# MariMamgo/CNN-with-PDE

Hardware: AMD Instinct MI355X
Metric: PDE-layer fwd+bwd Msamples/s (higher is better)
Workload: dtype f32; 1 GPU; cifar10.EnhancedDiffusionLayer(size=32, channels=64, num_steps=10) fwd+bwd, 30 implicit sweeps, batch 512/GPU, channel mixing disabled (BASELINE configs[1], SURVEY §8d cfg2 primary); global_batch=512, parallelism=dp1, grad_allreduce_bytes=0, rccl_world_size=1

## Files before the change

### cnn-with-pde_amd/_lib.py

```python
import ctypes as C
import os

HERE = os.path.dirname(os.path.abspath(__file__))
LIB_PATH = os.environ.get("PDECNN_LIB") or os.path.join(HERE, "lib", "libpdecnn_hip.so")

PDE_MAX_SWEEPS = 96
PDE_MAX_N = 32
PDE_MAX_N_GENERIC = 128
PDE_IO_F32, PDE_IO_BF16, PDE_IO_F64, PDE_IO_F16 = 0, 1, 2, 3
PDE_AXIS_X, PDE_AXIS_Y = 0, 1
PDE_MIX_PATH_SCALAR, PDE_MIX_PATH_MFMA_F32, PDE_MIX_PATH_MFMA_16, PDE_MIX_PATH_SPLIT3, PDE_MIX_PATH_FUSED = 0, 1, 2, 3, 4
PDE_RH_PATH_STRIP32, PDE_RH_PATH_STRIP16, PDE_RH_PATH_ROW_BLOCKS = 0, 1, 2
PDE_RH_DK_SPLIT3, PDE_RH_DK_MFMA_F32 = 0, 1
PDE_JACOBI_MAX_HW = 1024
PDE_JACOBI_TILED_K = 10

ERRORS = {
    -1: "PDE_E_BADARG (null pointer, bad dimension or enum)",
    -2: "PDE_E_UNSUPPORTED_N (line length — either side of a rectangle — outside [2, 128], or a per-step / one-launch "
        "entry point at a line length without fused kernels: those exist for multiples of 4 in [8, 32])",
    -3: "PDE_E_TOO_MANY_SWEEPS",
    -4: "PDE_E_LAUNCH (HIP launch failed)",
    -5: "PDE_E_WORKSPACE (workspace too small or misaligned)",
}


class PdeSweep(C.Structure):
    _fields_ = [("axis", C.c_int32), ("delta", C.c_float), ("h2", C.c_float), ("t", C.c_float)]


class PdeAdiDesc(C.Structure):
    _fields_ = [("B", C.c_int32), ("C", C.c_int32), ("N", C.c_int32), ("io_dtype", C.c_int32),
                ("num_sweeps", C.c_int32), ("smooth3", C.c_int32), ("has_clamp_max", C.c_int32),
                ("clamp_max", C.c_float), ("eps", C.c_float), ("sweep", PdeSweep * PDE_MAX_SWEEPS)]


class PdeSweepF64(C.Structure):
    _fields_ = [("axis", C.c_int32), ("pad", C.c_int32), ("delta", C.c_double), ("h2", C.c_double), ("t", C.c_double)]


class PdeAdiDescF64(C.Structure):
    _fields_ = [("B", C.c_int32), ("C", C.c_int32), ("N", C.c_int32), ("io_dtype", C.c_int32),
                ("num_sweeps", C.c_int32), ("smooth3", C.c_int32), ("has_clamp_max", C.c_int32), ("pad", C.c_int32),
                ("clamp_max", C.c_double), ("eps", C.c_double), ("sweep", PdeSweepF64 * PDE_MAX_SWEEPS)]


class PdeAdiRectDesc(C.Structure):
    _fields_ = [("B", C.c_int32), ("C", C.c_int32), ("H", C.c_int32), ("W", C.c_int32), ("io_dtype", C.c_int32),
                ("num_sweeps", C.c_int32), ("smooth3", C.c_int32), ("has_clamp_max", C.c_int32),
                ("clamp_max", C.c_float), ("eps", C.c_float), ("sweep", PdeSweep * PDE_MAX_SWEEPS)]


class PdeAdiRectDescF64(C.Structure):
    _fields_ = [("B", C.c_int32), ("C", C.c_int32), ("H", C.c_int32), ("W", C.c_int32), ("io_dtype", C.c_int32),
                ("num_sweeps", C.c_int32), ("smooth3", C.c_int32), ("has_clamp_max", C.c_int32),
                ("clamp_max", C.c_double), ("eps", C.c_double), ("sweep", PdeSweepF64 * PDE_MAX_SWEEPS)]


class PdeSmallLayer(C.Structure):
    _fields_ = [("desc", C.POINTER(PdeAdiDesc)), ("sweeps_per_step", C.c_int32), ("mode", C.c_int32),
                ("M", C.c_void_p), ("skip_weight", C.c_void_p),
                ("alpha_base", C.c_void_p), ("beta_base", C.c_void_p), ("alpha_slope", C.c_void_p), ("beta_slope", C.c_void_p),
                ("weight", C.c_float), ("weight_ptr", C.c_void_p), ("states", C.c_void_p), ("plane_sums", C.c_void_p),
                ("steps_workspace", C.c_void_p), ("steps_workspace_bytes", C.c_size_t),
                ("kappa_max", C.c_void_p), ("kappa_max_host", C.c_void_p),
                ("gys", C.c_void_p), ("g_plane_sums", C.c_void_p), ("ckpt_mask", C.POINTER(C.c_uint64)),
                ("g_alpha_base", C.c_void_p), ("g_beta_base", C.c_void_p), ("g_alpha_slope", C.c_void_p),
                ("g_beta_slope", C.c_void_p), ("gM", C.c_void_p), ("g_skip_weight", C.c_void_p), ("g_weight", C.c_void_p),
                ("workspace", C.c_void_p), ("workspace_bytes", C.c_size_t)]


class PdeError(RuntimeError):
    pass


_vp, _fp, _sz, _i32, _f32, _f64 = C.c_void_p, C.c_void_p, C.c_size_t, C.c_int32, C.c_float, C.c_double
_D = C.POINTER(PdeAdiDesc)
_D64 = C.POINTER(PdeAdiDescF64)
_DR = C.POINTER(PdeAdiRectDesc)
_DR64 = C.POINTER(PdeAdiRectDescF64)

SIGNATURES = {
    "pde_adi_line_length_path": (C.c_int, [_i32]),
    "pde_adi_forward_kernel": (C.c_int, [C.POINTER(PdeAdiDesc)]),
    "pde_adi_backward_kernel": (C.c_int, [C.POINTER(PdeAdiDesc), _i32]),
    "pde_adi_forward_workspace_bytes": (_sz, [_D]),
    "pde_adi_backward_workspace_bytes": (_sz, [_D, _i32]),
    "pde_adi_forward": (C.c_int, [_D, _vp, _vp, _fp, _fp, _fp, _fp, _fp, _fp, _vp, _vp, _sz, _vp]),
    "pde_adi_backward": (C.c_int, [_D, _vp, _vp, _vp, C.POINTER(C.c_uint64), _vp, _fp, _fp, _fp, _fp,
                                   _fp, _fp, _fp, _fp, _vp, _vp, _sz, _vp]),
    "pde_adi_forward_states": (C.c_int, [_D, _vp, _vp, _vp, C.POINTER(C.c_uint64), _fp, _fp, _fp, _fp, _fp, _fp, _vp, _vp,
                                         _sz, _vp]),
    "pde_adi_backward_states": (C.c_int, [_D, _vp, _vp, C.POINTER(C.c_uint64), _vp, _vp, C.POINTER(C.c_uint64), _vp,
                                          _fp, _fp, _fp, _fp, _fp, _fp, _fp, _fp, _vp, _vp, _sz, _vp]),
    "pde_adi_kappa_max": (C.c_int, [_D, _fp, _fp, _fp, _fp, _fp, _vp]),
    "pde_adi_steps_workspace_bytes": (_sz, [_D, _i32]),
    "pde_adi_factor_steps": (C.c_int, [_D, _i32, _fp, _fp, _fp, _fp, _fp, _vp, _sz, _vp]),
    "pde_adi_forward_step": (C.c_int, [_D, _i32, _i32, _vp, _vp, _vp, _vp]),
    "pde_adi_backward_step_workspace_bytes": (_sz, [_D, _i32, _i32]),
    "pde_adi_backward_step": (C.c_int, [_D, _i32, _i32, _vp, _vp, _vp, C.POINTER(C.c_uint64), _vp, _vp, _vp, _sz,
                                        _i32, _vp]),
    "pde_adi_param_grads": (C.c_int, [_D, _i32, _fp, _fp, _fp, _fp, _fp, _fp, _fp, _fp, _vp, _vp, _vp]),
    "pde_adi_mixed_forward": (C.c_int, [_D, _i32, _i32, _vp, _vp, _vp, _fp, _fp, _fp, _fp, _fp, _fp, _fp, _vp, _vp, _sz, _vp]),
    "pde_adi_mixed_backward_workspace_bytes": (_sz, [_D, _i32, _i32]),
    "pde_adi_mixed_backward": (C.c_int, [_D, _i32, _i32, _vp, _vp, _vp, _vp, _fp, C.POINTER(C.c_uint64), _vp, _fp, _fp, _fp, _fp,
                                         _fp, _fp, _fp, _fp, _fp, _vp, _vp, _sz, _vp]),
    "pde_adi_small_supported": (C.c_int, [_D, _i32]),
    "pde_adi_mixed_one_launch": (C.c_int, [_D, _i32]),
    "pde_adi_small_forward": (C.c_int, [_D, _i32, _i32, _vp, _vp, _vp, _fp, _fp, _fp, _fp, _fp, _fp, _fp, _fp, _vp, _vp, _sz,
                                        _vp]),
    "pde_adi_small_backward_workspace_bytes": (_sz, [_D, _i32, _i32]),
    "pde_adi_small_backward": (C.c_int, [_D, _i32, _i32, _vp, _vp, _vp, _fp, _fp, C.POINTER(C.c_uint64), _vp,
                                         _fp, _fp, _fp, _fp, _fp, _fp, _fp, _fp, _fp, _fp, _vp, _vp, _sz, _vp]),
    "pde_adi_small_forward_states": (C.c_int, [_D, _i32, _i32, _vp, _vp, _vp, _vp, C.POINTER(C.c_uint64), _fp, _fp, _fp, _fp,
                                               _fp, _fp, _fp, _vp, _vp, _sz, _vp]),
    "pde_adi_small_backward_states": (C.c_int, [_D, _i32, _i32, _vp, _vp, C.POINTER(C.c_uint64), _vp, _vp, _fp,
                                                C.POINTER(C.c_uint64), _vp, _fp, _fp, _fp, _fp, _fp, _fp, _fp, _fp, _fp,
                                                _vp, _vp, _sz, _vp]),
    "pde_adi_multi_forward": (C.c_int, [_i32, C.POINTER(PdeSmallLayer), _vp, _vp, _vp, _vp]),
    "pde_adi_multi_backward": (C.c_int, [_i32, C.POINTER(PdeSmallLayer), _vp, _vp, _vp, _vp]),
    "pde_gate_combine_forward": (C.c_int, [_i32, _i32, _i32, _i32, _i32, C.POINTER(C.c_void_p), C.POINTER(C.c_void_p), _fp,
                                           _vp, _vp]),
    "pde_gate_combine_backward": (C.c_int, [_i32, _i32, _i32, _i32, _i32, _vp, C.POINTER(C.c_void_p), C.POINTER(C.c_void_p),
                                            _fp, C.POINTER(C.c_void_p), C.POINTER(C.c_void_p), _vp]),
    "pde_bn_pool_workspace_bytes": (_sz, [_i32, _i32]),
    "pde_bn_pool_forward": (C.c_int, [_i32, _i32, _i32, _fp, _fp, _fp, _f32, _i32, _f32, _fp, _fp, _fp, _fp, _fp, _vp, _vp, _sz,
                                      _vp]),
    "pde_bn_pool_backward": (C.c_int, [_i32, _i32, _i32, _fp, _fp, _fp, _fp, _vp, _fp, _i32, _fp, _fp, _fp, _vp, _sz, _vp]),
    "pde_channel_mix_forward": (C.c_int, [_i32, _i32, _i32, _i32, _vp, _fp, _vp, _vp]),
    "pde_channel_mix_backward_workspace_bytes": (_sz, [_i32, _i32, _i32]),
    "pde_channel_mix_backward": (C.c_int, [_i32, _i32, _i32, _i32, _vp, _vp, _fp, _vp, _fp, _vp, _sz, _vp]),
    "pde_channel_mix_backward_steps": (C.c_int, [_i32, _i32, _i32, _i32, _vp, _vp, _fp, _vp, _fp, _vp, _sz, _i32, _i32,
                                                 _vp]),
    "pde_channel_mix_path": (C.c_int, [_i32, _i32, _i32, _i32, _i32]),
    "pde_channel_mix_splits": (C.c_int, [_i32, _i32, _i32, _i32, _i32, C.POINTER(C.c_int64)]),
    "pde_skip_blend_forward": (C.c_int, [C.c_int64, _i32, _vp, _vp, _fp, _vp, _vp]),
    "pde_skip_blend_backward_workspace_bytes": (_sz, [C.c_int64]),
    "pde_skip_blend_backward": (C.c_int, [C.c_int64, _i32, _vp, _vp, _vp, _fp, _vp, _vp, _fp, _vp, _sz, _vp]),
    "pde_explicit5_forward": (C.c_int, [_i32, _i32, _i32, _i32, _i32, _vp, _fp, _fp, _f32, _f32, _f32, _f32, _i32, _vp,
                                        _vp, _vp]),
    "pde_explicit5_backward_workspace_bytes": (_sz, [_i32, _i32, _i32, _i32, _i32, _i32]),
    "pde_explicit5_backward": (C.c_int, [_i32, _i32, _i32, _i32, _i32, _vp, _vp, _vp, _fp, _fp, _f32, _f32, _f32, _f32,
                                         _i32, _vp, _fp, _fp, _vp, _sz, _vp]),
    "pde_jacobi_forward": (C.c_int, [_i32, _i32, _i32, _i32, _fp, _fp, _fp, _fp, _vp]),
    "pde_jacobi_backward_workspace_bytes": (_sz, [_i32, _i32, _i32, _i32]),
    "pde_jacobi_backward": (C.c_int, [_i32, _i32, _i32, _i32, _fp, _fp, _fp, _fp, _fp, _fp, _fp, _vp, _sz, _vp]),
    "pde_jacobi_plane_path": (C.c_int, [_i32, _i32]),
    "pde_jacobi_forward_workspace_bytes": (_sz, [_i32, _i32, _i32, _i32]),
    "pde_jacobi_io_forward_ws": (C.c_int, [_i32, _i32, _i32, _i32, _i32, _vp, _fp, _fp, _vp, _vp, _sz, _vp]),
    "pde_jacobi_io_forward": (C.c_int, [_i32, _i32, _i32, _i32, _i32, _vp, _fp, _fp, _vp, _vp]),
    "pde_jacobi_io_backward_workspace_bytes": (_sz, [_i32, _i32, _i32, _i32, _i32]),
    "pde_jacobi_io_backward": (C.c_int, [_i32, _i32, _i32, _i32, _i32, _vp, _vp, _fp, _fp, _vp, _fp, _fp, _vp, _sz, _vp]),
    "pde_jacobi_io_forward_states": (C.c_int, [_i32, _i32, _i32, _i32, _i32, _vp, _fp, _fp, _vp, _vp, C.POINTER(C.c_uint64),
                                               _vp, _sz, _vp]),
    "pde_jacobi_io_backward_states": (C.c_int, [_i32, _i32, _i32, _i32, _i32, _vp, _vp, _vp, C.POINTER(C.c_uint64), _fp, _fp,
                                                _vp, _fp, _fp, _vp, _sz, _vp]),
    "pde_explicit5_forward_states": (C.c_int, [_i32, _i32, _i32, _i32, _i32, _vp, _fp, _fp, _f32, _f32, _f32, _f32, _i32, _vp,
                                               _vp, _vp, C.POINTER(C.c_uint64), _vp]),
    "pde_explicit5_backward_states": (C.c_int, [_i32, _i32, _i32, _i32, _i32, _vp, _vp, _vp, _vp, C.POINTER(C.c_uint64), _fp,
                                                _fp, _f32, _f32, _f32, _f32, _i32, _vp, _fp, _fp, _vp, _sz, _vp]),
    "pde_sym_layer_supported": (C.c_int, [_i32, _i32]),
    "pde_sym_layer_workspace_bytes": (_sz, [_i32, _i32]),
    "pde_sym_layer_forward": (C.c_int, [_i32, _i32, _i32, _i32, _fp, _fp, _fp, _fp, _fp, _fp, _f32, _f32, _fp, _f32,
                                        _fp, _fp, _fp, _fp, _fp, _vp, _sz, _vp]),
    "pde_sym_layer_backward": (C.c_int, [_i32, _i32, _i32, _i32, _fp, _f32, _fp, _fp, _fp, _fp, _fp, _fp, _fp,
                                         _fp, _fp, _fp, _fp, _fp, _vp, _sz, _vp]),
    "pde_sym_layer_path": (C.c_int, [_i32, _i32, _i32, C.POINTER(C.c_int32), C.POINTER(C.c_int32), C.POINTER(C.c_int32)]),
    "pde_sym_layer_dk_path": (C.c_int, [_i32, _i32]),
    "pde_sym_layer_f16_supported": (C.c_int, [_i32, _i32]),
    "pde_sym_layer_f16_workspace_bytes": (_sz, [_i32, _i32]),
    "pde_sym_k_to_f16": (C.c_int, [_i32, _fp, _vp, _vp]),
    "pde_sym_layer_f16_forward": (C.c_int, [_i32, _i32, _i32, _i32, _fp, _vp, _fp, _fp, _fp, _fp, _f32, _f32, _fp, _f32,
                                            _vp, _vp, _fp, _fp, _vp, _vp, _sz, _vp]),
    "pde_sym_layer_f16_backward": (C.c_int, [_i32, _i32, _i32, _i32, _fp, _f32, _fp, _vp, _fp, _vp, _vp, _fp, _fp,
                                             _vp, _fp, _fp, _fp, _fp, _vp, _sz, _vp]),
    "pde_sym_layer_bf16_supported": (C.c_int, [_i32, _i32]),
    "pde_sym_layer_bf16_workspace_bytes": (_sz, [_i32, _i32]),
    "pde_sym_k_to_bf16": (C.c_int, [_i32, _fp, _vp, _vp]),
# ... 109 lines not shown
```

### cnn-with-pde_amd/csrc/pde_adi.hip

```cpp
#include "pde_adi_dev.h"
#include "pde_adi_small.h"
#include "pde_adi_wide.h"
#include "pde_adi_launch.h"
#include "pde_adi_gen.h"
#include "pde_adi_asm.h"

#include <cmath>
#include <cstdlib>
#include <cstring>
#include <mutex>
#include <type_traits>
#include <vector>

namespace pde {

Timing& timing() {
    static Timing t;
    return t;
}

int ensure_dynamic_lds(const void* kernel, int bytes, unsigned long long& done) {
    static std::mutex mu;
    int dev = 0;
    if (hipGetDevice(&dev) != hipSuccess || dev < 0 || dev >= 64) return PDE_E_LAUNCH;
    std::lock_guard<std::mutex> lk(mu);
    if (!((done >> dev) & 1ull)) {
        if (hipFuncSetAttribute(kernel, hipFuncAttributeMaxDynamicSharedMemorySize, bytes) != hipSuccess) return PDE_E_LAUNCH;
        done |= 1ull << dev;
    }
    return PDE_OK;
}

namespace {

struct FactorArgs {
    SweepTab* tab;
    int* varying;
    float t_first[2];
    const float* ab;
    const float* bb;
    const float* as;
    const float* bs;
    float* coef;
    float* wide;
    float* kmax;
    int C, N, S;
    int win;
    int smooth3, has_max;
    float cmax, eps;
    PdeSweep sweep[PDE_MAX_SWEEPS];
};

template <int N>
__device__ __forceinline__ void store_half_row(float* row, int hf, const float (&v)[N / 2]) {
    float h[kHalfPad];
#pragma unroll
    for (int k = 0; k < kHalfPad; ++k) h[k] = 0.f;
#pragma unroll
    for (int k = 0; k < N / 2; ++k) h[k] = v[k];
    float4* dst = reinterpret_cast<float4*>(row + hf * kHalfPad);
#pragma unroll
    for (int q = 0; q < kHalfPad / 4; ++q) dst[q] = make_float4(h[4 * q], h[4 * q + 1], h[4 * q + 2], h[4 * q + 3]);
    if (hf) *reinterpret_cast<float4*>(row + 2 * kHalfPad) = make_float4(0.f, 0.f, 0.f, 0.f);
}

__device__ __forceinline__ float clamp_theta(float th, const FactorArgs& a, bool& pass) {
    pass = (th >= a.eps) && (!a.has_max || th <= a.cmax);
    th = fmaxf(th, a.eps);
    if (a.has_max) th = fminf(th, a.cmax);
    return th;
}

constexpr int kFacLd = PDE_MAX_N + 1;
__host__ __device__ inline int flag_ints(int C) { return (C + 63) / 64 * 64; }

template <int N>
__global__ __launch_bounds__(128) void adi_factor_kernel(FactorArgs a) {
    constexpr int m = N / 2;
    __shared__ float fsm[2 * 2 * kFacLd * PDE_MAX_N];
    __shared__ __attribute__((aligned(16))) float rsm[2 * kRecStride];
    const int pairs = (a.C + 1) / 2;
    const int s = blockIdx.x / pairs;
    const int c = 2 * (blockIdx.x % pairs) + (threadIdx.x >> 6);
    const int hf = (threadIdx.x >> 5) & 1, line = threadIdx.x & 31;
    if (blockIdx.x == 0 && threadIdx.x < a.S) {
        const int idx = threadIdx.x;
        const int w = idx / a.win, loc = idx % a.win, lo = w * a.win;
        SweepTab* tab = a.tab + w;
        float tprev = 0.f, tlast = 0.f;
        int first = -1;
        const int ax = a.sweep[idx].axis;
        for (int q = lo; q < lo + a.win; ++q) {
            if (a.sweep[q].axis != ax) continue;
            if (first < 0) first = q - lo;
            if (q < idx) tprev = a.sweep[q].t;
            tlast = a.sweep[q].t;
        }
        tab->ysc[loc] = powf(1.0f + a.eps, -(float)(a.win - 1 - loc));
        tab->axis[loc] = ax;
        tab->dts[loc] = a.sweep[idx].t - tprev;
        tab->first_s[ax] = first;
        tab->t_last[ax] = tlast;
        if (loc == 0) {
            const int other = 1 - ax;
            bool seen = false;
            for (int q = lo; q < lo + a.win; ++q) seen |= (a.sweep[q].axis == other);
            if (!seen) { tab->first_s[other] = -1; tab->t_last[other] = 0.f; }
        }
    }
    float kmax_lane = 0.f;
    int any_differs_w = 0;
    const PdeSweep sw = a.sweep[s];
    const bool xax = sw.axis == PDE_AXIS_X;
    if (c < a.C) {
        float* rec = rsm + (threadIdx.x >> 6) * kRecStride;
        float* grec = a.coef + ((size_t)s * a.C + c) * kRecStride;
        float zero[m];
#pragma unroll
        for (int k = 0; k < m; ++k) zero[k] = 0.f;
        const bool idle = line >= N;
        const int ln = idle ? N - 1 : line;
        const float* base = xax ? a.ab : a.bb;
        const float* slope = xax ? a.as : a.bs;
        const size_t cbase = (size_t)c * N * N;
        const float third = 1.0f / 3.0f;
        const float one_eps = 1.0f + a.eps, r1e = 1.0f / one_eps;
        float* TH = fsm + (threadIdx.x >> 6) * (2 * kFacLd * PDE_MAX_N);
        float* PS = TH + kFacLd * PDE_MAX_N;
        bool differs = false;
        {
            const int wl = threadIdx.x & 63;
            const float4* b4 = reinterpret_cast<const float4*>(base + cbase);
            const float4* s4 = reinterpret_cast<const float4*>(slope + cbase);
            for (int f = wl; f < N * N / 4; f += 64) {
                const float4 bv = b4[f], sv = s4[f];
                const int hh = (4 * f) / N, ww = (4 * f) % N;
                const float bb[4] = {bv.x, bv.y, bv.z, bv.w}, ss[4] = {sv.x, sv.y, sv.z, sv.w};
#pragma unroll
                for (int q = 0; q < 4; ++q) {
                    bool ps, ps0;
                    const float t = clamp_theta(bb[q] + ss[q] * sw.t, a, ps);
                    (void)clamp_theta(bb[q] + ss[q] * a.t_first[sw.axis], a, ps0);
                    differs |= (ps != ps0);
                    TH[hh * kFacLd + ww + q] = t;
                    PS[hh * kFacLd + ww + q] = ps ? 1.0f : 0.0f;
                }
            }
        }
        __builtin_amdgcn_wave_barrier();
        float th[m + 1], pass[m];
#pragma unroll
        for (int k = 0; k <= m; ++k) {
            const int i = hf ? N - 1 - k : k;
            const int at = xax ? ln * kFacLd + i : i * kFacLd + ln;
            th[k] = TH[at];
            if (k < m) pass[k] = PS[at];
        }
        any_differs_w = __any(differs ? 1 : 0) != 0 ? 1 : 0;
        float kap[m];
        if (a.smooth3) {
#pragma unroll
            for (int k = 0; k < m; ++k) {
                const float outer = th[k > 0 ? k - 1 : 0];
                const float inner = th[k + 1];
                const float prev = hf ? inner : outer, nxt = hf ? outer : inner;
                kap[k] = (prev * third + th[k] * third) + nxt * third;
            }
        } else {
#pragma unroll
            for (int k = 0; k < m; ++k) kap[k] = th[k];
        }
#pragma unroll
        for (int k = 0; k < m; ++k) {
            kap[k] = (kap[k] * sw.delta) / sw.h2;
            if (!idle) kmax_lane = fmaxf(kmax_lane, kap[k]);
        }
        float inv[m], ee[m], invb[m];
        {
            float e = 0.f;
#pragma unroll
            for (int k = 0; k < m; ++k) {
                const float kp = kap[k];
                const float b = (k == 0) ? 1.0f + kp : 1.0f + 2.0f * kp;
                const float den = (b - kp * e) + a.eps;
                const float iv = 1.0f / den;
                e = kp * iv;
                inv[k] = iv;
                invb[k] = iv * one_eps;
                ee[k] = e;
            }
        }
        const float e_other = __shfl_xor(ee[m - 1], 32, 64);
        const float e_lo = hf ? e_other : ee[m - 1], e_hi = hf ? ee[m - 1] : e_other;
        if (hf == 0) rec[kG_Jn + line] = idle ? 0.f : 1.0f / (1.0f - e_lo * e_hi);
        float* row = rec + line * kLineStride;
        store_half_row<N>(row + kG_Inv, hf, idle ? zero : inv);
        store_half_row<N>(row + kG_E, hf, idle ? zero : ee);
        store_half_row<N>(row + kG_InvB, hf, idle ? zero : invb);
        float kx[m], mx[m];
        if (xax) {
#pragma unroll
            for (int k = 0; k < m; ++k) { kx[k] = kap[k] * r1e; mx[k] = pass[k]; }
        } else {
            const int h = ln;
            const int hm = h > 0 ? h - 1 : 0, hp = h + 1 < N ? h + 1 : N - 1;
#pragma unroll
            for (int k = 0; k < m; ++k) {
                const int w = hf ? N - 1 - k : k;
                float t0 = TH[h * kFacLd + w];
                if (a.smooth3) t0 = (TH[hm * kFacLd + w] * third + t0 * third) + TH[hp * kFacLd + w] * third;
                kx[k] = ((t0 * sw.delta) / sw.h2) * r1e;
                mx[k] = PS[h * kFacLd + w];
            }
        }
        store_half_row<N>(row + kG_KapX, hf, idle ? zero : kx);
        store_half_row<N>(row + kG_MaskX, hf, idle ? zero : mx);
        if (a.wide != nullptr) {
            float* wr = a.wide + ((size_t)s * a.C + c) * kWideRec;
            const int wl = threadIdx.x & 63;
            if (hf == 0) wr[kW_Jn + line] = idle ? 0.f : 1.0f / (1.0f - e_lo * e_hi);
            auto put = [&](int off, const float (&v)[m]) __attribute__((always_inline)) {
                float4* dst = reinterpret_cast<float4*>(wr + off) + wl;
#pragma unroll
                for (int q = 0; q < 4; ++q) {
                    float4 x;
                    x.x = (4 * q < m && !idle) ? v[4 * q < m ? 4 * q : 0] : 0.f;
                    x.y = (4 * q + 1 < m && !idle) ? v[4 * q + 1 < m ? 4 * q + 1 : 0] : 0.f;
                    x.z = (4 * q + 2 < m && !idle) ? v[4 * q + 2 < m ? 4 * q + 2 : 0] : 0.f;
                    x.w = (4 * q + 3 < m && !idle) ? v[4 * q + 3 < m ? 4 * q + 3 : 0] : 0.f;
                    dst[q * 64] = x;
                }
            };
            put(kW_Inv, inv); put(kW_E, ee); put(kW_InvB, invb); put(kW_KapX, kx);
        }
        __builtin_amdgcn_wave_barrier();
        static_assert(kRecStride % 4 == 0, "record is a whole number of 16-byte pieces");
        const float4* src = reinterpret_cast<const float4*>(rec);
        float4* dst = reinterpret_cast<float4*>(grec);
        for (int f = threadIdx.x & 63; f < kRecStride / 4; f += 64) dst[f] = src[f];
    }
    if (a.varying && c < a.C) {
        for (int o = 32; o > 0; o >>= 1) kmax_lane = fmaxf(kmax_lane, __shfl_xor(kmax_lane, o, 64));
        if ((threadIdx.x & 63) == 0) {
            int* dpart = a.varying + flag_ints(a.C);
            float* kpart = reinterpret_cast<float*>(dpart + (size_t)a.S * a.C);
            dpart[(size_t)s * a.C + c] = any_differs_w;
            kpart[(size_t)s * a.C + c] = kmax_lane;
        }
    }
}

__global__ __launch_bounds__(64) void adi_flags_kernel(int* varying, float* kmax, float* kmax_mapped, int S, int C) {
    const int* dpart = varying + flag_ints(C);
    const float* kpart = reinterpret_cast<const float*>(dpart + (size_t)S * C);
    const int lane = threadIdx.x, b = blockIdx.x;
    if (b < S) {
        if (kmax == nullptr) return;
        float m = 0.f;
        for (int c = lane; c < C; c += 64) m = fmaxf(m, kpart[(size_t)b * C + c]);
        for (int o = 32; o > 0; o >>= 1) m = fmaxf(m, __shfl_xor(m, o, 64));
        if (lane == 0) {
            kmax[b] = m;
            if (kmax_mapped) kmax_mapped[b] = m;
        }
    } else {
        const int c = b - S;
        int f = 0;
        for (int s = lane; s < S; s += 64) f |= dpart[(size_t)s * C + c];
        f = __any(f) ? 1 : 0;
        if (lane == 0) varying[c] = f;
    }
}

__global__ __launch_bounds__(64) void adi_kmax_kernel(FactorArgs a) {
    const int N = a.N;
    const int pairs = (a.C + 1) / 2;
    const int s = blockIdx.x / pairs;
    const int c = 2 * (blockIdx.x % pairs) + (threadIdx.x >> 5);
    const int line = threadIdx.x & 31;
    float km = 0.f;
    if (c < a.C && line < N) {
        const PdeSweep sw = a.sweep[s];
        const bool xax = sw.axis == PDE_AXIS_X;
        const float* base = xax ? a.ab : a.bb;
        const float* slope = xax ? a.as : a.bs;
        const size_t cbase = (size_t)c * N * N;
        const int st = xax ? 1 : N;
        const int o0 = xax ? line * N : line;
        float th[PDE_MAX_N];
        for (int i = 0; i < N; ++i) {
            float v = base[cbase + o0 + i * st] + slope[cbase + o0 + i * st] * sw.t;
            v = fmaxf(v, a.eps);
            if (a.has_max) v = fminf(v, a.cmax);
            th[i] = v;
        }
        const float third = 1.0f / 3.0f;
        for (int i = 0; i < N; ++i) {
            float v = th[i];
            if (a.smooth3) v = (th[i > 0 ? i - 1 : 0] * third + th[i] * third) + th[i + 1 < N ? i + 1 : N - 1] * third;
            km = fmaxf(km, (v * sw.delta) / sw.h2);
        }
    }
    for (int o = 32; o > 0; o >>= 1) km = fmaxf(km, __shfl_xor(km, o, 64));
    if (threadIdx.x == 0) atomicMax((unsigned int*)&a.kmax[s], __float_as_uint(km));
}

struct PgradArgs {
    const float* part;
    const float* ab;
    const float* bb;
    const float* as;
    const float* bs;
    float* g_ab;
    float* g_bb;
    float* g_as;
    float* g_bs;
    const int* varying;
    int C, N, S, G;
    int smooth3, has_max, accumulate;
    float cmax, eps;
    float wx, wy;
    float t_first[2];
    int have_axis[2];
    const float* gm_part;
    float* gM;
    float* g_skip;
    float* g_w;
    const float* skip_w;
    int gm_blocks;
};

__global__ __launch_bounds__(1024) void adi_pgrad_kernel(PgradArgs a) {
    __shared__ float sm[PDE_MAX_N][PDE_MAX_N + 1];
    const int N = a.N;
    const int tid = threadIdx.x;
    if ((int)blockIdx.x == 4 * a.C) {
        const int lane = tid & 63, wv = tid >> 6, nout = a.C * a.C + 2;
        for (int o = wv; o < nout; o += 16) {
            double sum = 0.0;
            if (o < a.C * a.C) {
                const int i = o / a.C, j = o % a.C;
                for (int g = lane; g < a.gm_blocks; g += 64) sum += a.gm_part[((size_t)g * a.C + i) * kGmStride + j];
            } else {
                const int col = (o == a.C * a.C) ? kSmallMaxC : kGmStride - 1;
                for (int g = lane; g < a.gm_blocks; g += 64)
                    for (int i = 0; i < a.C; ++i) sum += a.gm_part[((size_t)g * a.C + i) * kGmStride + col];
            }
            for (int x = 32; x > 0; x >>= 1) sum += __shfl_xor(sum, x, 64);
            if (lane == 0) {
                if (o < a.C * a.C) a.gM[o] = (float)sum;
                else if (o == a.C * a.C) {
                    if (a.g_skip != nullptr) {
                        const double sg = 1.0 / (1.0 + exp(-(double)*a.skip_w));
                        *a.g_skip = (float)((1.0 - sg) * sum);
                    }
                } else if (a.g_w != nullptr) *a.g_w = (float)sum;
            }
        }
        return;
    }
    const int c = blockIdx.x >> 2, arr = blockIdx.x & 3, ax = arr >> 1;
    const int h = tid / N, w = tid % N;
    const bool act = tid < N * N;
    if (act) {
        const int e = h * kLineStride + half_pos(w, N);
        const size_t gs = (size_t)a.C * 4 * kImage;
        const float* p0 = a.part + ((size_t)c * 4 + arr) * kImage + e;
        float s[8];
#pragma unroll
        for (int q = 0; q < 8; ++q) s[q] = 0.f;
        int g = 0;
        for (; g + 8 <= a.G; g += 8) {
#pragma unroll
            for (int q = 0; q < 8; ++q) s[q] += p0[(size_t)(g + q) * gs];
        }
        for (; g < a.G; ++g) s[0] += p0[(size_t)g * gs];
        sm[h][w] = ((s[0] + s[1]) + (s[2] + s[3])) + ((s[4] + s[5]) + (s[6] + s[7]));
    }
    __syncthreads();
    if (!act) return;
    const size_t off = ((size_t)c * N + h) * N + w;
    const float wgt = -(ax == 0 ? a.wx : a.wy);
    float gv;
    if (a.varying[c]) {
        gv = sm[h][w] * (a.smooth3 ? wgt * (1.0f / 3.0f) : wgt);
    } else if (a.smooth3) {
        const int i = (ax == 0) ? w : h;
        auto at = [&](int ii) { return (ax == 0) ? sm[h][ii] : sm[ii][w]; };
        const float cj = (i == 0 || i == N - 1) ? 2.0f : 1.0f;
        float sa = at(i) * cj;
        if (i > 0) sa += at(i - 1);
        if (i < N - 1) sa += at(i + 1);
        gv = sa * (1.0f / 3.0f) * wgt;
    } else {
        gv = sm[h][w] * wgt;
    }
    if (!a.varying[c]) {
        const float base = (ax == 0 ? a.ab : a.bb)[off];
        const float slope = (ax == 0 ? a.as : a.bs)[off];
        const float th = base + slope * a.t_first[ax];
        const bool pass = (th >= a.eps) && (!a.has_max || th <= a.cmax);
        if (!pass || !a.have_axis[ax]) gv = 0.f;
    }
    float* o = (arr == 0) ? a.g_ab : (arr == 1) ? a.g_as : (arr == 2) ? a.g_bb : a.g_bs;
    if (a.accumulate) o[off] += gv;
    else o[off] = gv;
}

size_t align_up(size_t x, size_t a) { return (x + a - 1) / a * a; }

bool fused_n(int N) { return N >= 8 && N <= PDE_MAX_N && (N % 4) == 0; }
int check_desc(const PdeAdiDesc* d, bool allow_generic = false) {
    if (!d) return PDE_E_BADARG;
    if (d->B <= 0 || d->C <= 0 || d->num_sweeps <= 0) return PDE_E_BADARG;
    if (!fused_n(d->N) && !(allow_generic && gen_n_ok(d->N))) return PDE_E_UNSUPPORTED_N;
    if (d->num_sweeps > PDE_MAX_SWEEPS) return PDE_E_TOO_MANY_SWEEPS;
    if (d->io_dtype != PDE_IO_F32 && d->io_dtype != PDE_IO_BF16 && d->io_dtype != PDE_IO_F16) return PDE_E_BADARG;
    for (int s = 0; s < d->num_sweeps; ++s)
        if (d->sweep[s].axis != PDE_AXIS_X && d->sweep[s].axis != PDE_AXIS_Y) return PDE_E_BADARG;
    return PDE_OK;
}

size_t coef_bytes(const PdeAdiDesc* d) {
    return align_up((size_t)d->num_sweeps * d->C * kRecStride * sizeof(float), 256);
}
size_t tab_bytes() { return align_up(sizeof(SweepTab), 256); }
size_t flag_bytes(const PdeAdiDesc* d) {
    return align_up(((size_t)flag_ints(d->C) + 2 * (size_t)d->num_sweeps * d->C) * sizeof(int), 256);
}


int env_int(const char* name, int dflt) {
    const char* v = getenv(name);
    return v ? atoi(v) : dflt;
}
bool use_xcd_map(const PdeAdiDesc* d) { return (d->C % 8) == 0 && env_int("PDE_XCD", 1) != 0; }
int groups_per_channel(const PdeAdiDesc* d, int planes_per_iter, int wg_per_cu) {
    if (wg_per_cu < 1) wg_per_cu = 1;
    const int nchunk = (d->B + planes_per_iter - 1) / planes_per_iter;
    int G = (256 * wg_per_cu + d->C - 1) / d->C;
    G = env_int(planes_per_iter == kWaves * kJBwd ? "PDE_G_BWD" : "PDE_G_FWD", G);
    if (G < 1) G = 1;
    if (G > nchunk) G = nchunk;
    return G;
}

void fill_factor_args(FactorArgs& fa, const PdeAdiDesc* d, const float* ab, const float* bb, const float* as,
                      const float* bs) {
    fa.tab = nullptr; fa.varying = nullptr; fa.coef = nullptr; fa.kmax = nullptr; fa.wide = nullptr;
    fa.ab = ab; fa.bb = bb; fa.as = as; fa.bs = bs;
    fa.C = d->C; fa.N = d->N; fa.S = d->num_sweeps; fa.win = d->num_sweeps;
    fa.smooth3 = d->smooth3; fa.has_max = d->has_clamp_max; fa.cmax = d->clamp_max; fa.eps = d->eps;
    fa.t_first[0] = fa.t_first[1] = 0.f;
    bool seen[2] = {false, false};
    for (int s = 0; s < d->num_sweeps; ++s) {
        fa.sweep[s] = d->sweep[s];
        const int ax = d->sweep[s].axis;
        if (!seen[ax]) { seen[ax] = true; fa.t_first[ax] = d->sweep[s].t; }
    }
}

float* mapped_host(float* host) {
    static const int allow = [] {
        const int e = env_int("PDE_KMAX_MAPPED", -1);
        if (e >= 0) return e;
        int n = 0;
        return (hipGetDeviceCount(&n) == hipSuccess && n == 1) ? 1 : 0;
    }();
    void* dp = nullptr;
    if (!allow || !host || hipHostGetDevicePointer(&dp, host, 0) != hipSuccess) { (void)hipGetLastError(); return nullptr; }
    return static_cast<float*>(dp);
}

int launch_factor(const PdeAdiDesc* d, const float* ab, const float* bb, const float* as, const float* bs,
                  float* coef, SweepTab* tab, int* varying, float* kmax, hipStream_t st, int window = 0,
                  float* kmax_mapped = nullptr, float* wide = nullptr) {
    FactorArgs fa;
    fill_factor_args(fa, d, ab, bb, as, bs);
    fa.coef = coef; fa.tab = tab; fa.varying = varying; fa.kmax = kmax; fa.wide = wide;
    if (window > 0) fa.win = window;
    const dim3 grid(d->num_sweeps * ((d->C + 1) / 2));
    switch (d->N) {
#define PDE_CASE(NN) case NN: hipLaunchKernelGGL(adi_factor_kernel<NN>, grid, dim3(128), 0, st, fa); break;
        PDE_CASE(8) PDE_CASE(12) PDE_CASE(16) PDE_CASE(20) PDE_CASE(24) PDE_CASE(28) PDE_CASE(32)
#undef PDE_CASE
        default: return PDE_E_UNSUPPORTED_N;
    }
    if (varying) hipLaunchKernelGGL(adi_flags_kernel, dim3(d->num_sweeps + d->C), dim3(64), 0, st, varying, kmax, kmax_mapped, d->num_sweeps, d->C);
    return check_launch();
}

struct PendingEvent { hipEvent_t e0, e1; bool fwd; };
std::vector<PendingEvent>& pending() {
    static std::vector<PendingEvent> v;
    return v;
}
std::mutex& launch_mutex() {
    static std::mutex m;
    return m;
}

int publish_kmax(const float* kmax_dev, float* kmax_host, void* event, int n, hipStream_t st, bool written = false) {
    if (kmax_host && !written) {
        if (!kmax_dev) return PDE_E_BADARG;
        if (hipMemcpyAsync(kmax_host, kmax_dev, (size_t)n * sizeof(float), hipMemcpyDeviceToHost, st) != hipSuccess)
            return PDE_E_LAUNCH;
    }
    if (event && hipEventRecord(static_cast<hipEvent_t>(event), st) != hipSuccess) return PDE_E_LAUNCH;
    return PDE_OK;
}

bool strang_pairs_identical(const PdeAdiDesc* d) {
    if (d->num_sweeps % 3) return false;
    for (int s = 2; s + 1 < d->num_sweeps; s += 3) {
        const PdeSweep &p = d->sweep[s], &q = d->sweep[s + 1];
        if (p.axis != PDE_AXIS_X || q.axis != PDE_AXIS_X || p.t != q.t || p.delta != q.delta || p.h2 != q.h2) return false;
    }
    return true;
}

int split_of(const PdeAdiDesc* d) {
    const int S = d->num_sweeps;
    bool strang = (S % 3) == 0, lie = (S % 2) == 0;
    for (int s = 0; s < S; ++s) {
        const int ax = d->sweep[s].axis;
        if (ax != ((s % 3) == 1 ? PDE_AXIS_Y : PDE_AXIS_X)) strang = false;
        if (ax != ((s % 2) == 1 ? PDE_AXIS_Y : PDE_AXIS_X)) lie = false;
    }
    return strang ? kSplitStrang : (lie ? kSplitLie : kSplitAny);
}

template <typename F>
int timed_launch(F&& f, hipStream_t st, bool is_fwd, bool timed) {
    Timing& tm = timing();
    hipEvent_t e0 = nullptr, e1 = nullptr;
    const bool rec = tm.on && timed;
    if (rec) {
        (void)hipEventCreate(&e0); (void)hipEventCreate(&e1);
        (void)hipEventRecord(e0, st);
    }
    const int rc = f();
    if (rec) {
        (void)hipEventRecord(e1, st);
        std::lock_guard<std::mutex> lk(launch_mutex());
        pending().push_back({e0, e1, is_fwd});
    }
    return rc;
}

#define PDE_N_LIST PDE_CASE(8) PDE_CASE(12) PDE_CASE(16) PDE_CASE(20) PDE_CASE(24) PDE_CASE(28) PDE_CASE(32)

int dispatch_fwd(const PdeAdiDesc* d, int split, const SweepArgs& sa, int grid, size_t lds, hipStream_t st,
                 bool timed = true, int ho = 0) {
    return timed_launch([&]() -> int {
        switch (d->N) {
#define PDE_CASE(NN) case NN: return adi_launch_fwd_##NN(d->io_dtype, split, ho, &sa, grid, lds, st);
            PDE_N_LIST
#undef PDE_CASE
        }
        return PDE_E_UNSUPPORTED_N;
    }, st, true, timed);
}

int dispatch_bwd(const PdeAdiDesc* d, int split, const SweepArgs& sa, int grid, hipStream_t st) {
    return timed_launch([&]() -> int {
        switch (d->N) {
// ... 843 lines not shown
}

int pde_adi_multi_backward(int32_t num_layers, const PdeSmallLayer* layers, const void* gy, const void* u, void* gu,
                           void* stream) {
    return small_backward_impl(num_layers, layers, gy, u, gu, stream, nullptr, nullptr);
}

int pde_adi_small_forward(const PdeAdiDesc* d, int32_t sweeps_per_step, int32_t mode, const void* u, void* y, void* states,
                          const float* M, const float* skip_weight, const float* alpha_base, const float* beta_base,
                          const float* alpha_slope, const float* beta_slope, float* kappa_max, float* kappa_max_host,
                          void* kappa_event, void* steps_workspace, size_t workspace_bytes, void* stream) {
    PdeSmallLayer l{};
    l.desc = d; l.sweeps_per_step = sweeps_per_step; l.mode = mode; l.M = M; l.skip_weight = skip_weight;
    l.alpha_base = alpha_base; l.beta_base = beta_base; l.alpha_slope = alpha_slope; l.beta_slope = beta_slope;
    l.weight = 1.0f; l.states = states; l.steps_workspace = steps_workspace; l.steps_workspace_bytes = workspace_bytes;
    l.kappa_max = kappa_max; l.kappa_max_host = kappa_max_host;
    return pde_adi_multi_forward(1, &l, u, y, kappa_event, stream);
}

int pde_adi_small_backward(const PdeAdiDesc* d, int32_t sweeps_per_step, int32_t mode, const void* gy, const void* u,
                           const void* states, const float* M, const float* skip_weight, const uint64_t ckpt_mask[2],
                           void* gu, const float* alpha_base, const float* beta_base, const float* alpha_slope,
                           const float* beta_slope, float* g_alpha_base, float* g_beta_base, float* g_alpha_slope,
                           float* g_beta_slope, float* gM, float* g_skip_weight, const void* steps_workspace,
                           void* workspace, size_t workspace_bytes, void* stream) {
    if (!gy) return PDE_E_BADARG;
    PdeSmallLayer l{};
    l.desc = d; l.sweeps_per_step = sweeps_per_step; l.mode = mode; l.M = M; l.skip_weight = skip_weight;
    l.alpha_base = alpha_base; l.beta_base = beta_base; l.alpha_slope = alpha_slope; l.beta_slope = beta_slope;
    l.weight = 1.0f; l.states = const_cast<void*>(states); l.steps_workspace = const_cast<void*>(steps_workspace);
    l.ckpt_mask = ckpt_mask; l.g_alpha_base = g_alpha_base; l.g_beta_base = g_beta_base; l.g_alpha_slope = g_alpha_slope;
    l.g_beta_slope = g_beta_slope; l.gM = gM; l.g_skip_weight = g_skip_weight; l.workspace = workspace;
    l.workspace_bytes = workspace_bytes;
    return pde_adi_multi_backward(1, &l, gy, u, gu, stream);
}

int pde_adi_small_forward_states(const PdeAdiDesc* d, int32_t sweeps_per_step, int32_t mode, const void* u, void* y,
                                 void* states, void* traj, const uint64_t emit_mask[2], const float* M,
                                 const float* alpha_base, const float* beta_base, const float* alpha_slope,
                                 const float* beta_slope, float* kappa_max, float* kappa_max_host, void* kappa_event,
                                 void* steps_workspace, size_t workspace_bytes, void* stream) {
    bool any;
    const int rc = small_emit_check(d, sweeps_per_step, traj, emit_mask, any);
    if (rc != PDE_OK) return rc;
    PdeSmallLayer l{};
    l.desc = d; l.sweeps_per_step = sweeps_per_step; l.mode = mode; l.M = M;
    l.alpha_base = alpha_base; l.beta_base = beta_base; l.alpha_slope = alpha_slope; l.beta_slope = beta_slope;
    l.weight = 1.0f; l.states = states; l.steps_workspace = steps_workspace; l.steps_workspace_bytes = workspace_bytes;
    l.kappa_max = kappa_max; l.kappa_max_host = kappa_max_host;
    return small_forward_impl(1, &l, u, y, kappa_event, stream, traj, any ? emit_mask : nullptr);
}

int pde_adi_small_backward_states(const PdeAdiDesc* d, int32_t sweeps_per_step, int32_t mode, const void* gy,
                                  const void* gtraj, const uint64_t emit_mask[2], const void* u, const void* states,
                                  const float* M, const uint64_t ckpt_mask[2], void* gu, const float* alpha_base,
                                  const float* beta_base, const float* alpha_slope, const float* beta_slope,
                                  float* g_alpha_base, float* g_beta_base, float* g_alpha_slope, float* g_beta_slope,
                                  float* gM, const void* steps_workspace, void* workspace, size_t workspace_bytes,
                                  void* stream) {
    bool any;
    const int rc = small_emit_check(d, sweeps_per_step, gtraj, emit_mask, any);
    if (rc != PDE_OK) return rc;
    if (!gy) return PDE_E_BADARG;
    PdeSmallLayer l{};
    l.desc = d; l.sweeps_per_step = sweeps_per_step; l.mode = mode; l.M = M;
    l.alpha_base = alpha_base; l.beta_base = beta_base; l.alpha_slope = alpha_slope; l.beta_slope = beta_slope;
    l.weight = 1.0f; l.states = const_cast<void*>(states); l.steps_workspace = const_cast<void*>(steps_workspace);
    l.ckpt_mask = ckpt_mask; l.g_alpha_base = g_alpha_base; l.g_beta_base = g_beta_base; l.g_alpha_slope = g_alpha_slope;
    l.g_beta_slope = g_beta_slope; l.gM = gM; l.workspace = workspace; l.workspace_bytes = workspace_bytes;
    return small_backward_impl(1, &l, gy, u, gu, stream, gtraj, any ? emit_mask : nullptr);
}

int pde_adi_kappa_max(const PdeAdiDesc* d, const float* alpha_base, const float* beta_base, const float* alpha_slope,
                      const float* beta_slope, float* kappa_max, void* stream) {
    int rc = check_desc(d, true);
    if (rc != PDE_OK) return rc;
    if (!alpha_base || !beta_base || !alpha_slope || !beta_slope || !kappa_max) return PDE_E_BADARG;
    hipStream_t st = static_cast<hipStream_t>(stream);
    if (!fused_n(d->N)) return gen_kappa_max(d, alpha_base, beta_base, alpha_slope, beta_slope, kappa_max, st);
    if (hipMemsetAsync(kappa_max, 0, (size_t)d->num_sweeps * sizeof(float), st) != hipSuccess) return PDE_E_LAUNCH;
    FactorArgs fa;
    fill_factor_args(fa, d, alpha_base, beta_base, alpha_slope, beta_slope);
    fa.kmax = kappa_max;
    hipLaunchKernelGGL(adi_kmax_kernel, dim3(d->num_sweeps * ((d->C + 1) / 2)), dim3(64), 0, st, fa);
    return check_launch();
}

int pde_timing_enable(int32_t on) {
    timing().on = on != 0;
    if (on) { timing().fwd_ms = timing().bwd_ms = 0; timing().fwd_n = timing().bwd_n = 0; }
    return PDE_OK;
}

int pde_timing_read(double* fwd_ms_sum, int64_t* fwd_launches, double* bwd_ms_sum, int64_t* bwd_launches) {
    std::lock_guard<std::mutex> lk(launch_mutex());
    for (auto& p : pending()) {
        float ms = 0.f;
        (void)hipEventSynchronize(p.e1);
        (void)hipEventElapsedTime(&ms, p.e0, p.e1);
        if (p.fwd) { timing().fwd_ms += ms; timing().fwd_n++; } else { timing().bwd_ms += ms; timing().bwd_n++; }
        (void)hipEventDestroy(p.e0); (void)hipEventDestroy(p.e1);
    }
    pending().clear();
    if (fwd_ms_sum) *fwd_ms_sum = timing().fwd_ms;
    if (fwd_launches) *fwd_launches = timing().fwd_n;
    if (bwd_ms_sum) *bwd_ms_sum = timing().bwd_ms;
    if (bwd_launches) *bwd_launches = timing().bwd_n;
    return PDE_OK;
}

const char* pde_version(void) { return "pdecnn-hip 0.4 (gfx950)"; }

}
```

### include/pdecnn.h

```cpp
#ifndef PDECNN_H
#define PDECNN_H

#include <stddef.h>
#include <stdint.h>

#ifdef __cplusplus
extern "C" {
#endif

#define PDE_MAX_SWEEPS 96
#define PDE_MAX_N 32
#define PDE_MAX_N_GENERIC 128

#define PDE_OK 0
#define PDE_E_BADARG (-1)
#define PDE_E_UNSUPPORTED_N (-2)
#define PDE_E_TOO_MANY_SWEEPS (-3)
#define PDE_E_LAUNCH (-4)
#define PDE_E_WORKSPACE (-5)

#define PDE_IO_F32 0
#define PDE_IO_BF16 1
#define PDE_IO_F64 2
#define PDE_IO_F16 3

#define PDE_AXIS_X 0
#define PDE_AXIS_Y 1

typedef struct PdeSweep {
    int32_t axis;
    float   delta;
    float   h2;
    float   t;
} PdeSweep;

typedef struct PdeAdiDesc {
    int32_t B, C, N;
    int32_t io_dtype;
    int32_t num_sweeps;
    int32_t smooth3;
    int32_t has_clamp_max;
    float   clamp_max;
    float   eps;
    PdeSweep sweep[PDE_MAX_SWEEPS];
} PdeAdiDesc;


int pde_adi_line_length_path(int32_t N);

int pde_adi_forward_kernel(const PdeAdiDesc* d);

int pde_adi_backward_kernel(const PdeAdiDesc* d, int32_t num_checkpoints);

size_t pde_adi_forward_workspace_bytes(const PdeAdiDesc* d);
size_t pde_adi_backward_workspace_bytes(const PdeAdiDesc* d, int32_t num_checkpoints);

int pde_adi_forward(const PdeAdiDesc* d, const void* u, void* y,
                    const float* alpha_base, const float* beta_base,
                    const float* alpha_slope, const float* beta_slope,
                    float* kappa_max, float* kappa_max_host, void* kappa_event,
                    void* workspace, size_t workspace_bytes, void* stream);

int pde_adi_backward(const PdeAdiDesc* d, const void* gy, const void* y, const void* u,
                     const uint64_t ckpt_mask[2], void* gu,
                     const float* alpha_base, const float* beta_base,
                     const float* alpha_slope, const float* beta_slope,
                     float* g_alpha_base, float* g_beta_base,
                     float* g_alpha_slope, float* g_beta_slope,
                     const void* fwd_workspace ,
                     void* workspace, size_t workspace_bytes, void* stream);

int pde_adi_forward_states(const PdeAdiDesc* d, const void* u, void* y, void* states, const uint64_t emit_mask[2],
                           const float* alpha_base, const float* beta_base,
                           const float* alpha_slope, const float* beta_slope,
                           float* kappa_max, float* kappa_max_host, void* kappa_event,
                           void* workspace, size_t workspace_bytes, void* stream);
int pde_adi_backward_states(const PdeAdiDesc* d, const void* gy, const void* gstates, const uint64_t emit_mask[2],
                            const void* y, const void* u, const uint64_t ckpt_mask[2], void* gu,
                            const float* alpha_base, const float* beta_base,
                            const float* alpha_slope, const float* beta_slope,
                            float* g_alpha_base, float* g_beta_base,
                            float* g_alpha_slope, float* g_beta_slope,
                            const void* fwd_workspace, void* workspace, size_t workspace_bytes, void* stream);

int pde_adi_kappa_max(const PdeAdiDesc* d,
                      const float* alpha_base, const float* beta_base,
                      const float* alpha_slope, const float* beta_slope,
                      float* kappa_max, void* stream);

size_t pde_adi_steps_workspace_bytes(const PdeAdiDesc* d, int32_t sweeps_per_step);
int pde_adi_factor_steps(const PdeAdiDesc* d, int32_t sweeps_per_step,
                         const float* alpha_base, const float* beta_base,
                         const float* alpha_slope, const float* beta_slope,
                         float* kappa_max, void* steps_workspace, size_t workspace_bytes, void* stream);
int pde_adi_forward_step(const PdeAdiDesc* d, int32_t sweeps_per_step, int32_t step,
                         const void* u, void* y, const void* steps_workspace, void* stream);
size_t pde_adi_backward_step_workspace_bytes(const PdeAdiDesc* d, int32_t sweeps_per_step, int32_t num_checkpoints);
int pde_adi_backward_step(const PdeAdiDesc* d, int32_t sweeps_per_step, int32_t step,
                          const void* gy, const void* y, const void* u, const uint64_t ckpt_mask[2], void* gu,
                          const void* steps_workspace, void* workspace, size_t workspace_bytes,
                          int32_t accumulate, void* stream);
int pde_adi_param_grads(const PdeAdiDesc* d, int32_t sweeps_per_step,
                        const float* alpha_base, const float* beta_base,
                        const float* alpha_slope, const float* beta_slope,
                        float* g_alpha_base, float* g_beta_base, float* g_alpha_slope, float* g_beta_slope,
                        const void* steps_workspace, const void* workspace, void* stream);

int pde_adi_mixed_one_launch(const PdeAdiDesc* d, int32_t sweeps_per_step);
int pde_adi_mixed_forward(const PdeAdiDesc* d, int32_t sweeps_per_step, int32_t mode,
                          const void* u, void* states,
                          void* y ,
                          const float* M,
                          const float* alpha_base, const float* beta_base,
                          const float* alpha_slope, const float* beta_slope,
                          float* kappa_max, float* kappa_max_host, void* kappa_event ,
                          void* steps_workspace, size_t workspace_bytes, void* stream);
size_t pde_adi_mixed_backward_workspace_bytes(const PdeAdiDesc* d, int32_t sweeps_per_step, int32_t num_checkpoints);
int pde_adi_mixed_backward(const PdeAdiDesc* d, int32_t sweeps_per_step, int32_t mode,
                           const void* gy, const void* u, const void* states, const void* y ,
                           const float* M,
                           const uint64_t ckpt_mask[2], void* gu,
                           const float* alpha_base, const float* beta_base,
                           const float* alpha_slope, const float* beta_slope,
                           float* g_alpha_base, float* g_beta_base, float* g_alpha_slope, float* g_beta_slope,
                           float* gM, const void* steps_workspace,
                           void* workspace, size_t workspace_bytes, void* stream);

int pde_adi_small_supported(const PdeAdiDesc* d, int32_t sweeps_per_step);
int pde_adi_small_forward(const PdeAdiDesc* d, int32_t sweeps_per_step, int32_t mode,
                          const void* u, void* y, void* states, const float* M, const float* skip_weight,
                          const float* alpha_base, const float* beta_base,
                          const float* alpha_slope, const float* beta_slope,
                          float* kappa_max, float* kappa_max_host, void* kappa_event,
                          void* steps_workspace, size_t workspace_bytes, void* stream);
size_t pde_adi_small_backward_workspace_bytes(const PdeAdiDesc* d, int32_t sweeps_per_step, int32_t num_checkpoints);
int pde_adi_small_backward(const PdeAdiDesc* d, int32_t sweeps_per_step, int32_t mode,
                           const void* gy, const void* u, const void* states, const float* M, const float* skip_weight,
                           const uint64_t ckpt_mask[2], void* gu,
                           const float* alpha_base, const float* beta_base,
                           const float* alpha_slope, const float* beta_slope,
                           float* g_alpha_base, float* g_beta_base, float* g_alpha_slope, float* g_beta_slope,
                           float* gM, float* g_skip_weight, const void* steps_workspace,
                           void* workspace, size_t workspace_bytes, void* stream);

int pde_adi_small_forward_states(const PdeAdiDesc* d, int32_t sweeps_per_step, int32_t mode,
                                 const void* u, void* y, void* states, void* traj, const uint64_t emit_mask[2],
                                 const float* M,
                                 const float* alpha_base, const float* beta_base,
                                 const float* alpha_slope, const float* beta_slope,
                                 float* kappa_max, float* kappa_max_host, void* kappa_event,
                                 void* steps_workspace, size_t workspace_bytes, void* stream);
int pde_adi_small_backward_states(const PdeAdiDesc* d, int32_t sweeps_per_step, int32_t mode,
                                  const void* gy, const void* gtraj, const uint64_t emit_mask[2],
                                  const void* u, const void* states, const float* M,
                                  const uint64_t ckpt_mask[2], void* gu,
                                  const float* alpha_base, const float* beta_base,
                                  const float* alpha_slope, const float* beta_slope,
                                  float* g_alpha_base, float* g_beta_base, float* g_alpha_slope, float* g_beta_slope,
                                  float* gM, const void* steps_workspace,
                                  void* workspace, size_t workspace_bytes, void* stream);

typedef struct PdeSmallLayer {
    const PdeAdiDesc* desc;
    int32_t sweeps_per_step;
    int32_t mode;
    const float* M;
    const float* skip_weight;
    const float* alpha_base; const float* beta_base; const float* alpha_slope; const float* beta_slope;
    float weight;
    const float* weight_ptr;
    void* states;
// ... 368 lines not shown
```

Before: 1.213 Msamples/s.

## Factor each distinct sweep record once and fan out to duplicate slots

Detects sweeps whose (axis, delta, h2, t) descriptors are byte-identical and launches the factor and kappa-max kernels only over the distinct representatives. Each representative's block then writes its tridiagonal factor records, wide records, flags and kappa max into every duplicate slot through a linked list. The factor kernel is templated on waves per block and runs one channel per 64-thread block by default to keep the grid large. This removes redundant factorisation work, at the cost of extra scattered global stores per block and a smaller, possibly less occupied grid.

```diff
diff --git a/cnn-with-pde_amd/_lib.py b/cnn-with-pde_amd/_lib.py
--- a/cnn-with-pde_amd/_lib.py
+++ b/cnn-with-pde_amd/_lib.py
@@ -94,6 +94,7 @@
     "pde_adi_backward_states": (C.c_int, [_D, _vp, _vp, C.POINTER(C.c_uint64), _vp, _vp, C.POINTER(C.c_uint64), _vp,
                                           _fp, _fp, _fp, _fp, _fp, _fp, _fp, _fp, _vp, _vp, _sz, _vp]),
     "pde_adi_kappa_max": (C.c_int, [_D, _fp, _fp, _fp, _fp, _fp, _vp]),
+    "pde_adi_distinct_records": (C.c_int, [_D, C.POINTER(C.c_int32)]),
     "pde_adi_steps_workspace_bytes": (_sz, [_D, _i32]),
     "pde_adi_factor_steps": (C.c_int, [_D, _i32, _fp, _fp, _fp, _fp, _fp, _vp, _sz, _vp]),
     "pde_adi_forward_step": (C.c_int, [_D, _i32, _i32, _vp, _vp, _vp, _vp]),
diff --git a/cnn-with-pde_amd/csrc/pde_adi.hip b/cnn-with-pde_amd/csrc/pde_adi.hip
--- a/cnn-with-pde_amd/csrc/pde_adi.hip
+++ b/cnn-with-pde_amd/csrc/pde_adi.hip
@@ -49,6 +49,9 @@
     int smooth3, has_max;
     float cmax, eps;
     PdeSweep sweep[PDE_MAX_SWEEPS];
+    int nrep;
+    unsigned char reps[PDE_MAX_SWEEPS];
+    signed char next[PDE_MAX_SWEEPS];
 };
 
 template <int N>
@@ -74,17 +77,16 @@
 constexpr int kFacLd = PDE_MAX_N + 1;
 __host__ __device__ inline int flag_ints(int C) { return (C + 63) / 64 * 64; }
 
-template <int N>
-__global__ __launch_bounds__(128) void adi_factor_kernel(FactorArgs a) {
+template <int N, int W>
+__global__ __launch_bounds__(64 * W) void adi_factor_kernel(FactorArgs a) {
     constexpr int m = N / 2;
-    __shared__ float fsm[2 * 2 * kFacLd * PDE_MAX_N];
-    __shared__ __attribute__((aligned(16))) float rsm[2 * kRecStride];
-    const int pairs = (a.C + 1) / 2;
-    const int s = blockIdx.x / pairs;
-    const int c = 2 * (blockIdx.x % pairs) + (threadIdx.x >> 6);
+    __shared__ float fsm[W * 2 * kFacLd * PDE_MAX_N];
+    __shared__ __attribute__((aligned(16))) float rsm[W * kRecStride];
+    const int per = (a.C + W - 1) / W;
+    const int s = a.reps[blockIdx.x / per];
+    const int c = W * (blockIdx.x % per) + (threadIdx.x >> 6);
     const int hf = (threadIdx.x >> 5) & 1, line = threadIdx.x & 31;
-    if (blockIdx.x == 0 && threadIdx.x < a.S) {
-        const int idx = threadIdx.x;
+    if (blockIdx.x == 0) for (int idx = threadIdx.x; idx < a.S; idx += 64 * W) {
         const int w = idx / a.win, loc = idx % a.win, lo = w * a.win;
         SweepTab* tab = a.tab + w;
         float tprev = 0.f, tlast = 0.f;
@@ -216,36 +218,51 @@
         store_half_row<N>(row + kG_KapX, hf, idle ? zero : kx);
         store_half_row<N>(row + kG_MaskX, hf, idle ? zero : mx);
         if (a.wide != nullptr) {
-            float* wr = a.wide + ((size_t)s * a.C + c) * kWideRec;
             const int wl = threadIdx.x & 63;
-            if (hf == 0) wr[kW_Jn + line] = idle ? 0.f : 1.0f / (1.0f - e_lo * e_hi);
-            auto put = [&](int off, const float (&v)[m]) __attribute__((always_inline)) {
-                float4* dst = reinterpret_cast<float4*>(wr + off) + wl;
+            const float jn = idle ? 0.f : 1.0f / (1.0f - e_lo * e_hi);
+            for (int t = s; t >= 0; t = a.next[t]) {
+                float* wr = a.wide + ((size_t)t * a.C + c) * kWideRec;
+                if (hf == 0) wr[kW_Jn + line] = jn;
+                auto put = [&](int off, const float (&v)[m]) __attribute__((always_inline)) {
+                    float4* dst = reinterpret_cast<float4*>(wr + off) + wl;
 #pragma unroll
-                for (int q = 0; q < 4; ++q) {
-                    float4 x;
-                    x.x = (4 * q < m && !idle) ? v[4 * q < m ? 4 * q : 0] : 0.f;
-                    x.y = (4 * q + 1 < m && !idle) ? v[4 * q + 1 < m ? 4 * q + 1 : 0] : 0.f;
-                    x.z = (4 * q + 2 < m && !idle) ? v[4 * q + 2 < m ? 4 * q + 2 : 0] : 0.f;
-                    x.w = (4 * q + 3 < m && !idle) ? v[4 * q + 3 < m ? 4 * q + 3 : 0] : 0.f;
-                    dst[q * 64] = x;
-                }
-            };
-            put(kW_Inv, inv); put(kW_E, ee); put(kW_InvB, invb); put(kW_KapX, kx);
+                    for (int q = 0; q < 4; ++q) {
+                        float4 x;
+                        x.x = (4 * q < m && !idle) ? v[4 * q < m ? 4 * q : 0] : 0.f;
+                        x.y = (4 * q + 1 < m && !idle) ? v[4 * q + 1 < m ? 4 * q + 1 : 0] : 0.f;
+                        x.z = (4 * q + 2 < m && !idle) ? v[4 * q + 2 < m ? 4 * q + 2 : 0] : 0.f;
+                        x.w = (4 * q + 3 < m && !idle) ? v[4 * q + 3 < m ? 4 * q + 3 : 0] : 0.f;
+                        dst[q * 64] = x;
+                    }
+                };
+                put(kW_Inv, inv); put(kW_E, ee); put(kW_InvB, invb); put(kW_KapX, kx);
+            }
         }
         __builtin_amdgcn_wave_barrier();
         static_assert(kRecStride % 4 == 0, "record is a whole number of 16-byte pieces");
         const float4* src = reinterpret_cast<const float4*>(rec);
         float4* dst = reinterpret_cast<float4*>(grec);
-        for (int f = threadIdx.x & 63; f < kRecStride / 4; f += 64) dst[f] = src[f];
+        const int twin = a.next[s];
+        if (twin < 0) {
+            for (int f = threadIdx.x & 63; f < kRecStride / 4; f += 64) dst[f] = src[f];
+        } else {
+            const ptrdiff_t slot4 = (ptrdiff_t)a.C * (kRecStride / 4);
+            for (int f = threadIdx.x & 63; f < kRecStride / 4; f += 64) {
+                const float4 v = src[f];
+                dst[f] = v;
+                for (int t = twin; t >= 0; t = a.next[t]) dst[(ptrdiff_t)(t - s) * slot4 + f] = v;
+            }
+        }
     }
     if (a.varying && c < a.C) {
         for (int o = 32; o > 0; o >>= 1) kmax_lane = fmaxf(kmax_lane, __shfl_xor(kmax_lane, o, 64));
         if ((threadIdx.x & 63) == 0) {
             int* dpart = a.varying + flag_ints(a.C);
             float* kpart = reinterpret_cast<float*>(dpart + (size_t)a.S * a.C);
-            dpart[(size_t)s * a.C + c] = any_differs_w;
-            kpart[(size_t)s * a.C + c] = kmax_lane;
+            for (int t = s; t >= 0; t = a.next[t]) {
+                dpart[(size_t)t * a.C + c] = any_differs_w;
+                kpart[(size_t)t * a.C + c] = kmax_lane;
+            }
         }
     }
 }
@@ -275,7 +292,7 @@
 __global__ __launch_bounds__(64) void adi_kmax_kernel(FactorArgs a) {
     const int N = a.N;
     const int pairs = (a.C + 1) / 2;
-    const int s = blockIdx.x / pairs;
+    const int s = a.reps[blockIdx.x / pairs];
     const int c = 2 * (blockIdx.x % pairs) + (threadIdx.x >> 5);
     const int line = threadIdx.x & 31;
     float km = 0.f;
@@ -302,7 +319,8 @@
         }
     }
     for (int o = 32; o > 0; o >>= 1) km = fmaxf(km, __shfl_xor(km, o, 64));
-    if (threadIdx.x == 0) atomicMax((unsigned int*)&a.kmax[s], __float_as_uint(km));
+    if (threadIdx.x == 0)
+        for (int t = s; t >= 0; t = a.next[t]) atomicMax((unsigned int*)&a.kmax[t], __float_as_uint(km));
 }
 
 struct PgradArgs {
@@ -445,8 +463,36 @@
     return G;
 }
 
+int distinct_records(const PdeAdiDesc* d, int32_t* rep) {
+    int n = 0;
+    for (int s = 0; s < d->num_sweeps; ++s) {
+        rep[s] = s;
+        for (int q = 0; q < s; ++q)
+            if (rep[q] == q && memcmp(&d->sweep[q], &d->sweep[s], sizeof(PdeSweep)) == 0) { rep[s] = q; break; }
+        n += rep[s] == s;
+    }
+    return n;
+}
+static_assert(sizeof(PdeSweep) == 16, "axis, delta, h2, t and no padding: compared as bytes");
+
+bool factor_once() {
+    const char* e = getenv("PDE_FACTOR_ONCE");
+    return !(e && e[0] == '0');
+}
+
 void fill_factor_args(FactorArgs& fa, const PdeAdiDesc* d, const float* ab, const float* bb, const float* as,
                       const float* bs) {
+    int32_t rep[PDE_MAX_SWEEPS];
+    if (factor_once()) (void)distinct_records(d, rep);
+    else for (int s = 0; s < d->num_sweeps; ++s) rep[s] = s;
+    fa.nrep = 0;
+    int last[PDE_MAX_SWEEPS];
+    for (int s = 0; s < d->num_sweeps; ++s) {
+        fa.next[s] = -1;
+        if (rep[s] == s) fa.reps[fa.nrep++] = (unsigned char)s;
+        else fa.next[last[rep[s]]] = (signed char)s;
+        last[rep[s]] = s;
+    }
     fa.tab = nullptr; fa.varying = nullptr; fa.coef = nullptr; fa.kmax = nullptr; fa.wide = nullptr;
     fa.ab = ab; fa.bb = bb; fa.as = as; fa.bs = bs;
     fa.C = d->C; fa.N = d->N; fa.S = d->num_sweeps; fa.win = d->num_sweeps;
@@ -479,9 +525,13 @@
     fill_factor_args(fa, d, ab, bb, as, bs);
     fa.coef = coef; fa.tab = tab; fa.varying = varying; fa.kmax = kmax; fa.wide = wide;
     if (window > 0) fa.win = window;
-    const dim3 grid(d->num_sweeps * ((d->C + 1) / 2));
+    const bool once = factor_once();
+    const dim3 grid(once ? fa.nrep * d->C : fa.nrep * ((d->C + 1) / 2));
     switch (d->N) {
-#define PDE_CASE(NN) case NN: hipLaunchKernelGGL(adi_factor_kernel<NN>, grid, dim3(128), 0, st, fa); break;
+#define PDE_CASE(NN) case NN: \
+        if (once) hipLaunchKernelGGL((adi_factor_kernel<NN, 1>), grid, dim3(64), 0, st, fa); \
+        else hipLaunchKernelGGL((adi_factor_kernel<NN, 2>), grid, dim3(128), 0, st, fa); \
+        break;
         PDE_CASE(8) PDE_CASE(12) PDE_CASE(16) PDE_CASE(20) PDE_CASE(24) PDE_CASE(28) PDE_CASE(32)
 #undef PDE_CASE
         default: return PDE_E_UNSUPPORTED_N;
@@ -1491,8 +1541,15 @@
     FactorArgs fa;
     fill_factor_args(fa, d, alpha_base, beta_base, alpha_slope, beta_slope);
     fa.kmax = kappa_max;
-    hipLaunchKernelGGL(adi_kmax_kernel, dim3(d->num_sweeps * ((d->C + 1) / 2)), dim3(64), 0, st, fa);
+    hipLaunchKernelGGL(adi_kmax_kernel, dim3(fa.nrep * ((d->C + 1) / 2)), dim3(64), 0, st, fa);
     return check_launch();
+}
+
+int pde_adi_distinct_records(const PdeAdiDesc* d, int32_t* rep) {
+    const int rc = check_desc(d, true);
+    if (rc != PDE_OK) return rc;
+    if (!rep) return PDE_E_BADARG;
+    return distinct_records(d, rep);
 }
 
 int pde_timing_enable(int32_t on) {
diff --git a/include/pdecnn.h b/include/pdecnn.h
--- a/include/pdecnn.h
+++ b/include/pdecnn.h
@@ -87,6 +87,8 @@
                       const float* alpha_base, const float* beta_base,
                       const float* alpha_slope, const float* beta_slope,
                       float* kappa_max, void* stream);
+
+int pde_adi_distinct_records(const PdeAdiDesc* d, int32_t* rep );
 
 size_t pde_adi_steps_workspace_bytes(const PdeAdiDesc* d, int32_t sweeps_per_step);
 int pde_adi_factor_steps(const PdeAdiDesc* d, int32_t sweeps_per_step,
```

Result: no change. 1.211 Msamples/s (-0.1%).
